# google/supersonic

Hardware: AMD Instinct MI355X
Metric: rows/sec filter->project->aggregate, 100M x 8 INT64/DOUBLE (higher is better)
Workload: dtype int64/f64; 1 GPU; Q-FPA-wide: SUM(a+b),COUNT(*),SUM(c),MIN(d),MAX(d0),SUM(d1),SUM(d2*d3) WHERE a>499 over a device-resident 100000000-row x 8-col block per GPU; rows_per_gpu=100000000, parallelism=single GPU, tile_rows=512, grid=768, lds_bytes=35568, specialized_stages=1

## Files before the change

### supersonic_amd/csrc/launch.h

```cpp
#ifndef SSGPU_LAUNCH_H_
#define SSGPU_LAUNCH_H_

#ifndef __HIPCC_RTC__
#include <hip/hip_runtime_api.h>
#include <stdint.h>
#endif
#include "vm.h"

enum SlotKind {
  SLOT_SUM_INT = 0, SLOT_SUM_DD = 1, SLOT_MIN_U64 = 2, SLOT_MAX_U64 = 3, SLOT_MIN_F64 = 4,
  SLOT_MAX_F64 = 5, SLOT_FIRST = 6, SLOT_LAST = 7, SLOT_COUNT = 8
};
enum EmitKind {
  EMIT_U64 = 0, EMIT_I64KEY = 1, EMIT_U32 = 2, EMIT_I32KEY = 3, EMIT_F64 = 4, EMIT_F32 = 5,
  EMIT_DD_F64 = 6, EMIT_DD_F32 = 7, EMIT_U8 = 8,
  EMIT_DDRES_F64 = 9,
  EMIT_CNT_U64 = 20, EMIT_CNT_U32 = 21,
  EMIT_FKEY_F64 = 100, EMIT_FKEY_F32 = 101
};
#define SSGPU_STATE_ARRAYS 8

struct EmitDesc { void* data; uint8_t* is_null; int slot; int out_kind; };

struct GroupKeyOut { void* data; uint8_t* is_null; uint32_t shift, bits, nullbit, width; };
// ... 129 lines not shown
  const unsigned char* key_nulls[8];
  unsigned int width[8], shift[8], bits[8];
  unsigned int n_keys;
  unsigned int capacity_mask;
  unsigned long long n_rows;
  unsigned long long* keys;
  unsigned int* rows;
  unsigned int* special;
  unsigned int* flags;
  unsigned int* counts;
  unsigned int* slot_of_row;
  unsigned int word[8];
  unsigned long long* keys_hi;
};
hipError_t ssgpu_launch_join_expand(const unsigned int* offsets, const unsigned int* run_start, const unsigned int* rows_sorted,
                                    unsigned long long n_lhs, unsigned long long n_out, unsigned int* lhs_idx, unsigned int* rhs_row, hipStream_t stream);
hipError_t ssgpu_launch_join_build(const JoinBuildParams& P, hipStream_t stream);
hipError_t ssgpu_launch_fill_u32(unsigned int* p, unsigned int v, size_t n, hipStream_t stream);
struct GroupInitParams {
  unsigned long long* keys; unsigned long long n_keys;
  unsigned long long* acc; const unsigned long long* pattern; unsigned int ng; unsigned long long n_acc;
  unsigned int* cnt; unsigned long long n_cnt;
  unsigned int* z[4]; unsigned long long nz[4];
  unsigned int n_rep, pad; unsigned long long rep_stride;
};
hipError_t ssgpu_launch_group_init(const GroupInitParams& P, hipStream_t stream);

hipError_t ssgpu_launch_pipeline(const VmParams& P, int K, int grid, hipStream_t stream);
#ifndef __HIPCC_RTC__
#include <string>
void* ssgpu_rtc_specialize(int device, const VmInstr* prog, int n_instr, int K, bool math, const uint32_t* staged_width, const uint32_t* staged_lds_off,
                           int n_staged, uint32_t static_lds, std::string* why);
hipError_t ssgpu_launch_pipeline_rtc(void* handle, const VmParams& P, int grid, bool static_lds, hipStream_t stream);
void* ssgpu_rtc_specialize_part_agg(int device, const unsigned long long* desc, int n_aggs, unsigned int rec_words, unsigned int n_gaggs, bool any_cnt,
                                    unsigned int lds_bytes, std::string* why, const PlainScatterParams* source = nullptr,
                                    bool dense = false,
                                    bool prefetch = false);
hipError_t ssgpu_launch_group_resident_rtc(void* handle, const PartAggParams& A, const PlainScatterParams& S, int grid, hipStream_t stream);
hipError_t ssgpu_launch_part_agg_rtc(void* handle, const PartAggParams& P, hipStream_t stream);
void* ssgpu_rtc_specialize_pscat(int device, const PlainScatterParams& S, const PscatGeom& g, std::string* why);
hipError_t ssgpu_launch_part_scatter_plain_rtc(void* handle, const PlainScatterParams& P, const PscatGeom& g, int grid, hipStream_t stream);
void* ssgpu_rtc_function(void* handle);
void ssgpu_rtc_release(void* handle);
void ssgpu_rtc_cached_only(bool on);
void ssgpu_rtc_mode(int mode);
int ssgpu_rtc_current_mode();
bool ssgpu_rtc_pending();
void ssgpu_rtc_trim(int keep);
void ssgpu_rtc_stats(long long* modules, long long* code_bytes, long long* compilations, long long* disk_hits);
#endif
hipError_t ssgpu_pipeline_set_max_lds(int bytes);
hipError_t ssgpu_launch_finish_slots(const VmAccRec* partials, int n_slots, int n_parts, const int* slot_kind,
                                     VmAccRec* out, uint64_t* state , hipStream_t stream,
                                     const EmitDesc* descs = nullptr, int n_out = 0 );
hipError_t ssgpu_launch_slots_to_state(const VmAccRec* recs, int n_slots, const int* slot_kind, uint64_t* state,
                                       hipStream_t stream);
hipError_t ssgpu_launch_fold_state(const uint64_t* images, int n_images, uint64_t* state, int n_slots, const int* slot_kind, hipStream_t stream);
hipError_t ssgpu_launch_fold_emit(const uint64_t* images, int n_images, uint64_t* state, int n_slots, const int* slot_kind, VmAccRec* recs,
                                  const EmitDesc* descs, int n_out, hipStream_t stream);
hipError_t ssgpu_launch_state_to_slots(const uint64_t* state, int n_slots, const int* slot_kind, VmAccRec* recs,
                                       hipStream_t stream);
hipError_t ssgpu_launch_emit_scalar(const VmAccRec* recs, const EmitDesc* descs, int n_out, hipStream_t stream);
hipError_t ssgpu_launch_scan_counts(const uint32_t* in, uint32_t* out, int n, uint64_t* total, hipStream_t stream);
hipError_t ssgpu_launch_group_count(const GroupExtractParams& P, uint32_t* tile_counts, hipStream_t stream);
hipError_t ssgpu_launch_group_extract_lb(const GroupExtractParams& P, unsigned long long* status, uint64_t epoch, unsigned int* ctrl, unsigned int* error_flag, hipStream_t stream);
hipError_t ssgpu_launch_group_extract(const GroupExtractParams& P, hipStream_t stream);
hipError_t ssgpu_launch_fill_u64(uint64_t* p, uint64_t v, size_t n, hipStream_t stream);
hipError_t ssgpu_launch_fill_pattern_u64(uint64_t* p, const uint64_t* pattern, uint32_t plen, size_t n,
                                         hipStream_t stream);

hipError_t ssgpu_launch_sort_iota(uint32_t* idx, uint64_t n, hipStream_t s);
hipError_t ssgpu_launch_sort_load_keys(uint64_t* keys, const uint32_t* idx, const void* col, const uint8_t* nulls, uint32_t width,
                                       int kind, int descending, int null_pass, uint64_t n, unsigned long long* bits, hipStream_t s);
uint32_t ssgpu_sort_tiles(uint64_t n);
hipError_t ssgpu_launch_sort_hist(const uint64_t* keys, uint32_t shift, uint64_t n, uint32_t* hist, hipStream_t s);
hipError_t ssgpu_launch_sort_scatter(const uint64_t* keys_in, const uint32_t* idx_in, uint64_t* keys_out, uint32_t* idx_out,
                                     uint32_t shift, uint64_t n, const uint32_t* offsets, hipStream_t s);
hipError_t ssgpu_launch_sort_load_keys_hist(uint64_t* keys, const uint32_t* idx, const void* col, const uint8_t* nulls, uint32_t width, int kind,
                                            int descending, int null_pass, uint64_t n, unsigned long long* bits, uint32_t* hist8, uint32_t* base8, hipStream_t s,
                                            uint64_t* compact_out = nullptr);
hipError_t ssgpu_launch_sort_onesweep(const uint64_t* keys_in, const uint32_t* idx_in, uint64_t* keys_out, uint32_t* idx_out, uint32_t shift, uint64_t n,
                                      const uint32_t* digit_base, unsigned long long* status, uint32_t* ticket, uint64_t epoch, uint32_t* stuck, hipStream_t s);
hipError_t ssgpu_launch_sort_fix_ties(uint64_t* keys, uint32_t* idx, uint64_t n, uint32_t hi_shift, uint32_t* too_long, hipStream_t s);
struct SortRecField { const void* src; void* dst; unsigned int off, width; };
#define SSGPU_SORT_MAX_FIELDS 96
struct SortRecParams { void* recs; unsigned long long n; unsigned int stride, n_fields; SortRecField fields[SSGPU_SORT_MAX_FIELDS]; };
hipError_t ssgpu_launch_sort_pack(const SortRecParams& P, hipStream_t s);
hipError_t ssgpu_launch_sort_gather_rec(const SortRecParams& P, const uint32_t* idx, uint32_t idx_stride, hipStream_t s);
hipError_t ssgpu_launch_sort_fix_ties_compact(uint64_t* kc, const uint64_t* keys, uint64_t n, uint32_t* too_long, hipStream_t s);
hipError_t ssgpu_launch_sort_extract_idx(uint32_t* idx, const uint64_t* kc, uint64_t n, hipStream_t s);
struct UnpackPiece { unsigned long long src_off; void* dst; unsigned long long bytes; };
hipError_t ssgpu_launch_unpack(const char* slab, const UnpackPiece* pieces, unsigned int n_pieces, hipStream_t s);
uint64_t ssgpu_str_scan_partials(uint64_t n);
hipError_t ssgpu_launch_str_scan(uint64_t* data, uint64_t n, uint64_t* partials, hipStream_t s);
hipError_t ssgpu_launch_str_hash(const uint8_t* bytes, const uint64_t* offs, const uint8_t* nulls, uint64_t n, uint64_t* hashes, hipStream_t s);
hipError_t ssgpu_launch_str_insert(const uint8_t* bytes, const uint64_t* offs, const uint8_t* nulls, const uint64_t* hashes, uint64_t n,
                                   uint64_t* table, uint64_t cap, uint32_t* row_slot, uint32_t* error, hipStream_t s);
hipError_t ssgpu_launch_str_compact(const uint64_t* table, uint64_t cap, const uint8_t* bytes, const uint64_t* offs, uint32_t* count,
                                    uint32_t* d_slot, uint64_t* d_off, uint64_t* d_len, uint64_t* d_key, uint32_t* d_idx, hipStream_t s);
hipError_t ssgpu_launch_str_sort(uint64_t* d_key, uint32_t* d_idx, uint64_t d, uint64_t p, const uint8_t* bytes, const uint64_t* d_off,
                                 const uint64_t* d_len, hipStream_t s);
hipError_t ssgpu_launch_str_rank(const uint32_t* d_idx, const uint32_t* d_slot, const uint64_t* d_len, uint64_t d, int32_t* slot_rank,
                                 uint64_t* out_len, hipStream_t s);
hipError_t ssgpu_launch_str_codes(const uint32_t* row_slot, const uint8_t* nulls, const int32_t* slot_rank, uint64_t n, int32_t* codes, hipStream_t s);
hipError_t ssgpu_launch_str_gather(const uint8_t* bytes, const uint64_t* d_off, const uint32_t* d_idx, const uint64_t* out_off, uint64_t d,
                                   uint8_t* out, hipStream_t s);
hipError_t ssgpu_launch_str_recode(const int32_t* src, const uint8_t* nulls, const int32_t* remap, int32_t n_remap, uint64_t n, int32_t* dst,
// ... 47 lines not shown
```

### supersonic_amd/csrc/pipeline_kernels.hip

```cpp
#ifndef __HIPCC_RTC__
#include <hip/hip_runtime.h>
#include <stdint.h>
#endif
#include "vm.h"
#include "launch.h"
#ifdef SSGPU_RTC_NINSTR
#include "rtc_prog.h"
#endif

typedef unsigned long long u64;
typedef long long i64;
typedef unsigned int u32;
typedef int i32;
typedef unsigned char u8;

#ifdef SSGPU_PC_PROFILE
#define PC_PROF(...) __VA_ARGS__
#else
#define PC_PROF(...)
#endif
struct LdsBase {
  __device__ __forceinline__ char* operator+(u32 off) const {
    return (char*)(__attribute__((address_space(3))) char*)off;
  }
// ... 679 lines not shown
        case SLOT_COUNT: v0 = cnt; break;
        case SLOT_SUM_INT: v0 = wave_reduce_u64(F0[s], [](u64 x, u64 y) { return x + y; }); break;
        case SLOT_MIN_U64: v0 = wave_reduce_u64(F0[s], [](u64 x, u64 y) { return x < y ? x : y; }); break;
        case SLOT_MAX_U64: v0 = wave_reduce_u64(F0[s], [](u64 x, u64 y) { return x > y ? x : y; }); break;
        case SLOT_MIN_F64: v0 = wave_reduce_u64(F0[s], [](u64 x, u64 y) { return u2d(y) < u2d(x) ? y : x; }); break;
        case SLOT_MAX_F64: v0 = wave_reduce_u64(F0[s], [](u64 x, u64 y) { return u2d(x) < u2d(y) ? y : x; }); break;
        case SLOT_SUM_DD: {
          DD d; d.hi = u2d(F0[s]); d.lo = u2d(F1[s]);
          d = wave_reduce_dd(d); v0 = d2u(d.hi); v1 = d2u(d.lo);
        } break;
        case SLOT_FIRST: case SLOT_LAST: {
          const bool first = kind == SLOT_FIRST;
          const u64 trow = first ? wave_reduce_u64(F1[s], [](u64 x, u64 y) { return x < y ? x : y; })
                                 : wave_reduce_u64(FC[s] ? F1[s] : 0ull, [](u64 x, u64 y) { return x > y ? x : y; });
          const u64 owner = __ballot(FC[s] != 0 && F1[s] == trow);
          const int src = owner ? __ffsll((long long)owner) - 1 : 0;
          v0 = readlane64(F0[s], src); v1 = trow;
        } break;
        default: break;
      }
      if (lane == 0) { VmAccRec* A = acc_rec(P, (u32)s, wave); A->v0 = v0; A->v1 = v1; A->cnt = cnt; A->pad = 0; }
    }
  }

  __syncthreads();
  for (int s = t; s < P.n_slots; s += VM_COMPUTE_THREADS)
    for (int w = 0; w < VM_WAVES; ++w)
      P.wg_partials[((size_t)blockIdx.x * P.n_slots + s) * VM_WAVES + w] = *acc_rec(P, (u32)s, w);
}
#endif

#ifndef __HIPCC_RTC__

__device__ __forceinline__ void combine_rec(int kind, VmAccRec& acc, const VmAccRec& r) {
  if (r.cnt == 0) return;
  switch (kind) {
    case SLOT_COUNT:
    case SLOT_SUM_INT: acc.v0 += r.v0; break;
    case SLOT_SUM_DD: {
      DD a; a.hi = u2d(acc.v0); a.lo = u2d(acc.v1);
      DD b; b.hi = u2d(r.v0); b.lo = u2d(r.v1);
      a = dd_add(a, b); acc.v0 = d2u(a.hi); acc.v1 = d2u(a.lo);
    } break;
    case SLOT_MIN_U64: acc.v0 = acc.cnt ? (r.v0 < acc.v0 ? r.v0 : acc.v0) : r.v0; break;
    case SLOT_MAX_U64: acc.v0 = acc.cnt ? (r.v0 > acc.v0 ? r.v0 : acc.v0) : r.v0; break;
    case SLOT_MIN_F64: acc.v0 = acc.cnt ? (u2d(r.v0) < u2d(acc.v0) ? r.v0 : acc.v0) : r.v0; break;
    case SLOT_MAX_F64: acc.v0 = acc.cnt ? (u2d(acc.v0) < u2d(r.v0) ? r.v0 : acc.v0) : r.v0; break;
    case SLOT_FIRST: if (!acc.cnt || r.v1 < acc.v1) { acc.v0 = r.v0; acc.v1 = r.v1; } break;
    case SLOT_LAST: if (!acc.cnt || r.v1 >= acc.v1) { acc.v0 = r.v0; acc.v1 = r.v1; } break;
  }
  acc.cnt += r.cnt;
}

__device__ __forceinline__ void slot_to_state(const VmAccRec r, int kind, int s, int n_slots, u64* __restrict__ state) {
  u64* sum_i = state; u64* cnt = state + n_slots; u64* hi = state + 2 * n_slots; u64* lo = state + 3 * n_slots;
  u64* mn = state + 4 * n_slots; u64* mx = state + 5 * n_slots;
  u64* mnf = state + 6 * n_slots; u64* mxf = state + 7 * n_slots;
  const bool fl = kind == SLOT_FIRST || kind == SLOT_LAST;
  sum_i[s] = (kind == SLOT_SUM_INT || kind == SLOT_COUNT || fl) ? r.v0 : 0;
  cnt[s] = r.cnt;
  hi[s] = kind == SLOT_SUM_DD ? r.v0 : d2u(0.0);
  lo[s] = kind == SLOT_SUM_DD ? r.v1 : d2u(0.0);
  mn[s] = (kind == SLOT_MIN_U64 && r.cnt) ? (r.v0 ^ 0x8000000000000000ull) : (kind == SLOT_FIRST && r.cnt) ? (r.v1 ^ 0x8000000000000000ull) : 0x7FFFFFFFFFFFFFFFull;
  mx[s] = (kind == SLOT_MAX_U64 && r.cnt) ? (r.v0 ^ 0x8000000000000000ull) : (kind == SLOT_LAST && r.cnt) ? (r.v1 ^ 0x8000000000000000ull) : 0x8000000000000000ull;
  mnf[s] = (kind == SLOT_MIN_F64 && r.cnt) ? r.v0 : d2u(__builtin_inf());
  mxf[s] = (kind == SLOT_MAX_F64 && r.cnt) ? r.v0 : d2u(-__builtin_inf());
}
__device__ __forceinline__ VmAccRec state_to_slot(const u64* __restrict__ state, int kind, int s, int n_slots) {
  VmAccRec r; r.v0 = 0; r.v1 = 0; r.pad = 0;
  r.cnt = state[n_slots + s];
  switch (kind) {
    case SLOT_COUNT: case SLOT_SUM_INT: r.v0 = state[s]; break;
    case SLOT_SUM_DD: {
      DD a; a.hi = u2d(state[2 * n_slots + s]); a.lo = 0.0;
      a = dd_add_d(a, u2d(state[3 * n_slots + s]));
      r.v0 = d2u(a.hi); r.v1 = d2u(a.lo);
    } break;
    case SLOT_MIN_U64: r.v0 = state[4 * n_slots + s] ^ 0x8000000000000000ull; break;
    case SLOT_MAX_U64: r.v0 = state[5 * n_slots + s] ^ 0x8000000000000000ull; break;
    case SLOT_MIN_F64: r.v0 = state[6 * n_slots + s]; break;
    case SLOT_MAX_F64: r.v0 = state[7 * n_slots + s]; break;
    case SLOT_FIRST: r.v0 = state[s]; r.v1 = state[4 * n_slots + s] ^ 0x8000000000000000ull; break;
    case SLOT_LAST: r.v0 = state[s]; r.v1 = state[5 * n_slots + s] ^ 0x8000000000000000ull; break;
    default: break;
  }
  return r;
}

__device__ __forceinline__ void emit_scalar_one(const EmitDesc d, const VmAccRec r);
__global__ __launch_bounds__(256) void ssgpu_finish_slots_kernel(const VmAccRec* __restrict__ partials, int n_slots,
                                                                 int n_parts, const int* __restrict__ slot_kind,
                                                                 VmAccRec* __restrict__ out, u64* __restrict__ state,
                                                                 const EmitDesc* __restrict__ descs, int n_out) {
  __shared__ VmAccRec tree[256];
  const int s = blockIdx.x, t = threadIdx.x;
  const int kind = slot_kind[s];
  VmAccRec acc; acc.v0 = 0; acc.v1 = 0; acc.cnt = 0; acc.pad = 0;
  if (kind == SLOT_SUM_DD) { acc.v0 = d2u(-0.0); acc.v1 = d2u(0.0); }
  for (int i = t; i < n_parts; i += 256) {
    const VmAccRec r = partials[((size_t)(i / VM_WAVES) * n_slots + s) * VM_WAVES + (i % VM_WAVES)];
    combine_rec(kind, acc, r);
  }
  tree[t] = acc;
  __syncthreads();
  for (int stride = 128; stride > 0; stride >>= 1) {
    if (t < stride) { VmAccRec a = tree[t]; combine_rec(kind, a, tree[t + stride]); tree[t] = a; }
    __syncthreads();
  }
  if (t == 0) { out[s] = tree[0]; if (state) slot_to_state(tree[0], kind, s, n_slots, state); }
  if (descs)
    for (int i = t; i < n_out; i += 256) { const EmitDesc d = descs[i]; if (d.slot == s) emit_scalar_one(d, tree[0]); }
}

__global__ void ssgpu_slots_to_state_kernel(const VmAccRec* __restrict__ recs, int n_slots,
                                            const int* __restrict__ slot_kind, u64* __restrict__ state) {
  int s = blockIdx.x * blockDim.x + threadIdx.x;
  if (s >= n_slots) return;
  slot_to_state(recs[s], slot_kind[s], s, n_slots, state);
}
__global__ void ssgpu_state_to_slots_kernel(const u64* __restrict__ state, int n_slots,
                                            const int* __restrict__ slot_kind, VmAccRec* __restrict__ recs) {
  int s = blockIdx.x * blockDim.x + threadIdx.x;
  if (s >= n_slots) return;
  recs[s] = state_to_slot(state, slot_kind[s], s, n_slots);
}


__device__ __forceinline__ void emit_value(void* dst, size_t idx, int out_kind, u64 v0, u64 v1) {
  switch (out_kind) {
    case EMIT_U64: reinterpret_cast<u64*>(dst)[idx] = v0; break;
    case EMIT_I64KEY: reinterpret_cast<i64*>(dst)[idx] = unkey_i64(v0); break;
    case EMIT_U32: reinterpret_cast<u32*>(dst)[idx] = (u32)v0; break;
    case EMIT_I32KEY: reinterpret_cast<i32*>(dst)[idx] = (i32)unkey_i64(v0); break;
    case EMIT_F64: reinterpret_cast<double*>(dst)[idx] = u2d(v0); break;
    case EMIT_F32: reinterpret_cast<float*>(dst)[idx] = (float)u2d(v0); break;
    case EMIT_DD_F64: { double hi = u2d(v0), lo = u2d(v1);
      reinterpret_cast<double*>(dst)[idx] = (lo == 0.0) ? hi : hi + lo; } break;
    case EMIT_DDRES_F64: { const double hi = u2d(v0), lo = u2d(v1), sm = hi + lo, bp = sm - hi;
      reinterpret_cast<double*>(dst)[idx] = (lo == 0.0) ? 0.0 : (hi - (sm - bp)) + (lo - bp); } break;
    case EMIT_DD_F32: { double hi = u2d(v0), lo = u2d(v1);
      reinterpret_cast<float*>(dst)[idx] = (float)((lo == 0.0) ? hi : hi + lo); } break;
    case EMIT_U8: reinterpret_cast<u8*>(dst)[idx] = (u8)(v0 != 0); break;
    default: break;
  }
}


__device__ __forceinline__ void emit_scalar_one(const EmitDesc d, const VmAccRec r) {
  if (d.out_kind == EMIT_CNT_U64 || d.out_kind == EMIT_CNT_U32)
    emit_value(d.data, 0, d.out_kind == EMIT_CNT_U64 ? EMIT_U64 : EMIT_U32, r.cnt, 0);
  else
    emit_value(d.data, 0, d.out_kind, r.v0, r.v1);
  if (d.is_null) d.is_null[0] = r.cnt == 0;
}
__global__ void ssgpu_emit_scalar_kernel(const VmAccRec* __restrict__ recs, const EmitDesc* __restrict__ descs,
                                         int n_out) {
  int i = blockIdx.x * blockDim.x + threadIdx.x;
  if (i >= n_out) return;
  const EmitDesc d = descs[i];
  emit_scalar_one(d, recs[d.slot]);
}

__global__ __launch_bounds__(1024) void ssgpu_scan_counts_kernel(const u32* __restrict__ in, u32* __restrict__ out,
                                                                  int n, u64* __restrict__ total) {
// ... 878 lines not shown
  }
  u64 bits;
  if (fam == 2) {
    const double tr = trunc(vf);
    bits = (tr >= -9223372036854775808.0 && tr < 9223372036854775808.0) ? (u64)(i64)tr : 0x8000000000000000ull;
  } else bits = fam == 1 ? vu : (u64)vi;
  if (dst_kind == 2 || dst_kind == 3) reinterpret_cast<u64*>(dst)[i] = bits;
  else if (dst_kind == 0 || dst_kind == 1) reinterpret_cast<u32*>(dst)[i] = (u32)bits;
  else reinterpret_cast<u8*>(dst)[i] = (u8)bits;
}
hipError_t ssgpu_launch_gather_rowid(void* dst, const uint8_t* dst_null, const void* src, uint32_t width, int src_kind, int dst_kind, const uint64_t* rowids, uint64_t rowid_mask,
                                     int64_t row_id_base, const uint64_t* n_rows_dev, uint64_t n_rows_max, hipStream_t stream) {
  if (n_rows_max) hipLaunchKernelGGL(ssgpu_gather_rowid_kernel, dim3((unsigned)((n_rows_max + 255) / 256)), dim3(256), 0, stream,
                                     dst, dst_null, src, width, src_kind, dst_kind, (const u64*)rowids, (u64)rowid_mask, (i64)row_id_base, (const u64*)n_rows_dev, (u64)n_rows_max);
  return hipGetLastError();
}
hipError_t ssgpu_launch_fill_u32(unsigned int* p, unsigned int v, size_t n, hipStream_t stream) {
  if (n) hipLaunchKernelGGL(ssgpu_fill_u32_kernel, dim3((unsigned)std::min<size_t>((n + 255) / 256, 4096)), dim3(256), 0, stream, p, v, n);
  return hipGetLastError();
}
hipError_t ssgpu_launch_part_agg(const PartAggParams& P, unsigned int lds_bytes, hipStream_t stream) {
  if (P.rec_words <= 8) hipLaunchKernelGGL(ssgpu_part_agg_kernel<8>, dim3(P.n_parts), dim3(SSGPU_PART_THREADS), lds_bytes, stream, P);
  else if (P.rec_words <= 16) hipLaunchKernelGGL(ssgpu_part_agg_kernel<16>, dim3(P.n_parts), dim3(SSGPU_PART_THREADS), lds_bytes, stream, P);
  else if (P.rec_words <= SSGPU_PART_MAX_WORDS) hipLaunchKernelGGL(ssgpu_part_agg_kernel<SSGPU_PART_MAX_WORDS>, dim3(P.n_parts), dim3(SSGPU_PART_THREADS), lds_bytes, stream, P);
  else return hipErrorInvalidValue;
  return hipGetLastError();
}
hipError_t ssgpu_launch_group_resident(const PartAggParams& P, const PlainScatterParams& S, unsigned int lds_bytes, int grid, hipStream_t stream) {
  if (P.rec_words <= 8) hipLaunchKernelGGL(ssgpu_group_resident_kernel<8>, dim3(grid), dim3(SSGPU_PART_THREADS), lds_bytes, stream, P, S);
  else hipLaunchKernelGGL(ssgpu_group_resident_kernel<16>, dim3(grid), dim3(SSGPU_PART_THREADS), lds_bytes, stream, P, S);
  return hipGetLastError();
}
hipError_t ssgpu_part_agg_set_max_lds(int bytes) {
  hipError_t e = hipFuncSetAttribute(reinterpret_cast<const void*>(ssgpu_part_agg_kernel<8>), hipFuncAttributeMaxDynamicSharedMemorySize, bytes);
  if (e != hipSuccess) return e;
  e = hipFuncSetAttribute(reinterpret_cast<const void*>(ssgpu_group_resident_kernel<8>), hipFuncAttributeMaxDynamicSharedMemorySize, bytes);
  if (e != hipSuccess) return e;
  e = hipFuncSetAttribute(reinterpret_cast<const void*>(ssgpu_group_resident_kernel<16>), hipFuncAttributeMaxDynamicSharedMemorySize, bytes);
  if (e != hipSuccess) return e;
  e = hipFuncSetAttribute(reinterpret_cast<const void*>(ssgpu_part_agg_kernel<SSGPU_PART_MAX_WORDS>), hipFuncAttributeMaxDynamicSharedMemorySize, bytes);
  if (e != hipSuccess) return e;
  return hipFuncSetAttribute(reinterpret_cast<const void*>(ssgpu_part_agg_kernel<16>), hipFuncAttributeMaxDynamicSharedMemorySize, bytes);
}
hipError_t ssgpu_pipeline_set_max_lds(int bytes) {
  hipError_t e;
  e = hipFuncSetAttribute(reinterpret_cast<const void*>(ssgpu_pipeline_kernel<1, false>), hipFuncAttributeMaxDynamicSharedMemorySize, bytes); if (e != hipSuccess) return e;
  e = hipFuncSetAttribute(reinterpret_cast<const void*>(ssgpu_pipeline_kernel<2, false>), hipFuncAttributeMaxDynamicSharedMemorySize, bytes); if (e != hipSuccess) return e;
  e = hipFuncSetAttribute(reinterpret_cast<const void*>(ssgpu_pipeline_kernel<4, false>), hipFuncAttributeMaxDynamicSharedMemorySize, bytes); if (e != hipSuccess) return e;
  e = hipFuncSetAttribute(reinterpret_cast<const void*>(ssgpu_pipeline_kernel<1, true>), hipFuncAttributeMaxDynamicSharedMemorySize, bytes); if (e != hipSuccess) return e;
  e = hipFuncSetAttribute(reinterpret_cast<const void*>(ssgpu_pipeline_kernel<2, true>), hipFuncAttributeMaxDynamicSharedMemorySize, bytes); if (e != hipSuccess) return e;
  e = hipFuncSetAttribute(reinterpret_cast<const void*>(ssgpu_pipeline_kernel<4, true>), hipFuncAttributeMaxDynamicSharedMemorySize, bytes);
  return e;
}
hipError_t ssgpu_launch_finish_slots(const VmAccRec* partials, int n_slots, int n_parts, const int* slot_kind,
                                     VmAccRec* out, uint64_t* state, hipStream_t stream, const EmitDesc* descs, int n_out) {
  hipLaunchKernelGGL(ssgpu_finish_slots_kernel, dim3(n_slots), dim3(256), 0, stream, partials, n_slots, n_parts, slot_kind, out, (u64*)state, descs, n_out);
  return hipGetLastError();
}
hipError_t ssgpu_launch_slots_to_state(const VmAccRec* recs, int n_slots, const int* slot_kind, uint64_t* state, hipStream_t stream) {
  int blocks = (n_slots + 63) / 64;
  hipLaunchKernelGGL(ssgpu_slots_to_state_kernel, dim3(blocks), dim3(64), 0, stream, recs, n_slots, slot_kind, (u64*)state);
  return hipGetLastError();
}
__device__ __forceinline__ void fold_state_slot(const u64* __restrict__ images, int n_images, u64* __restrict__ state, int n_slots, int kind, int s);
__global__ __launch_bounds__(64) void ssgpu_fold_state_kernel(const u64* __restrict__ images, int n_images, u64* __restrict__ state,
                                                              int n_slots, const int* __restrict__ slot_kind) {
  const int s = blockIdx.x * 64 + threadIdx.x;
  if (s >= n_slots) return;
  fold_state_slot(images, n_images, state, n_slots, slot_kind[s], s);
}
__device__ __forceinline__ void fold_state_slot(const u64* __restrict__ images, int n_images, u64* __restrict__ state, int n_slots, int kind, int s) {
  const size_t total = (size_t)SSGPU_STATE_ARRAYS * n_slots;
  u64 a[SSGPU_STATE_ARRAYS];
  for (int k = 0; k < SSGPU_STATE_ARRAYS; ++k) a[k] = images[(size_t)k * n_slots + s];
  for (int r = 1; r < n_images; ++r) {
    u64 v[SSGPU_STATE_ARRAYS];
    for (int k = 0; k < SSGPU_STATE_ARRAYS; ++k) v[k] = images[(size_t)r * total + (size_t)k * n_slots + s];
    if (kind == SLOT_FIRST) { if ((i64)v[4] < (i64)a[4]) a[0] = v[0]; }
    else if (kind == SLOT_LAST) { if ((i64)v[5] > (i64)a[5]) a[0] = v[0]; }
    else a[0] += v[0];
    a[1] += v[1];
    a[2] = d2u(u2d(a[2]) + u2d(v[2]));
    a[3] = d2u(u2d(a[3]) + u2d(v[3]));
    a[4] = (i64)v[4] < (i64)a[4] ? v[4] : a[4];
    a[5] = (i64)v[5] > (i64)a[5] ? v[5] : a[5];
    a[6] = u2d(v[6]) < u2d(a[6]) ? v[6] : a[6];
    a[7] = u2d(v[7]) > u2d(a[7]) ? v[7] : a[7];
  }
  for (int k = 0; k < SSGPU_STATE_ARRAYS; ++k) state[(size_t)k * n_slots + s] = a[k];
}
__global__ __launch_bounds__(256) void ssgpu_fold_emit_kernel(const u64* __restrict__ images, int n_images, u64* __restrict__ state, int n_slots,
                                                              const int* __restrict__ slot_kind, VmAccRec* __restrict__ recs,
                                                              const EmitDesc* __restrict__ descs, int n_out) {
  for (int s = threadIdx.x; s < n_slots; s += 256) {
    fold_state_slot(images, n_images, state, n_slots, slot_kind[s], s);
    recs[s] = state_to_slot(state, slot_kind[s], s, n_slots);
  }
  __threadfence_block();
  __syncthreads();
  for (int i = threadIdx.x; i < n_out; i += 256) { const EmitDesc d = descs[i]; emit_scalar_one(d, recs[d.slot]); }
}
hipError_t ssgpu_launch_fold_emit(const uint64_t* images, int n_images, uint64_t* state, int n_slots, const int* slot_kind, VmAccRec* recs,
                                  const EmitDesc* descs, int n_out, hipStream_t stream) {
  hipLaunchKernelGGL(ssgpu_fold_emit_kernel, dim3(1), dim3(256), 0, stream, (const u64*)images, n_images, (u64*)state, n_slots, slot_kind, recs, descs, n_out);
  return hipGetLastError();
}
hipError_t ssgpu_launch_fold_state(const uint64_t* images, int n_images, uint64_t* state, int n_slots, const int* slot_kind, hipStream_t stream) {
  if (n_slots > 0) hipLaunchKernelGGL(ssgpu_fold_state_kernel, dim3((n_slots + 63) / 64), dim3(64), 0, stream, (const u64*)images, n_images, (u64*)state, n_slots, slot_kind);
  return hipGetLastError();
// ... 94 lines not shown
```

### supersonic_amd/csrc/runtime.cpp

```cpp
#include <hip/hip_runtime_api.h>

#include <atomic>
#include <map>
#include <mutex>
#include <stdio.h>
#include <string.h>
#include <algorithm>
#include <cmath>
#include <string>
#include <unistd.h>
#include <thread>
#include <unordered_set>
#include <vector>
#include <deque>
#include <functional>

#include "engine.h"

using namespace ssgpu;

#define HIP_TRY(ctx, expr)                                                          \
  do {                                                                               \
    hipError_t _e = (expr);                                                          \
    if (_e != hipSuccess) {                                                          \
// ... 177 lines not shown
  std::vector<VmInstr> host_prog_main;
  std::string rtc_why;
  ProgramLayout lay{};
  ProgramLayout lay_count{};
  int n_instr_main = 0, n_instr_count = 0;
  int grid = 0;
  DevBuf wg_partials, slot_recs, slot_kind, emit_descs, state;
  DevBuf tile_counts, tile_offsets, total;
  DevBuf xstatus; uint64_t x_epoch = 0;
  DevBuf gkeys, gacc, gcnt, goverflow, gpattern, gmergeop;
  int group_wgs = 3;
  bool group_local = true;
  int group_sub = 1;
  bool group_partitioned = false;
  uint32_t part_n = 256;
  bool part_n_chosen = false;
  bool part_slab_failed = false;
  bool scouted = false;
  int64_t scout_full_rows = 0;
  bool part_slab = false;
  double part_groups_est = 0;
  uint32_t part_seg_growth = 1;
  bool part_failed = false;
  DevBuf prog_pscatter, part_hist, part_recs;
  ProgramLayout lay_pscatter{};
  int n_instr_pscatter = 0;
  RtcSlot rtc_pscatter; std::vector<VmInstr> host_prog_pscatter;
  RtcSlot rtc_plain;
  RtcSlot rtc_part;
  RtcSlot rtc_resident;
  RtcSlot rtc_hot;
  uint32_t hot_n = 0; uint64_t hot_keys[SSGPU_HOT_MAX] = {0};
  int64_t hot_sampled_run = -1;
  DevBuf hot_out;
  struct DenseState {
    bool on = false, failed = false, checked = false, fixed = false, resident = false;
    uint32_t n_keys = 0, n_chunks = 1;
    uint64_t lo[8] = {0}, hi[8] = {0};
    uint32_t span[8] = {0}, stride[8] = {0};
    uint64_t slots = 0;
    uint32_t np = 0, cap = 0;
    uint64_t chunk_bytes = 0;
    int64_t widened = 0;
  } dense;
  DevBuf dense_dom, dense_flags;
  void* dense_table = nullptr;
  std::vector<DevBuf> rowid_tmp;
  std::vector<DevBuf> jkeys, jkeys_hi, jrows, jmisc;
  std::vector<DevBuf> jcounts, jstarts, jslot_of_row, jrows_sorted;
  DevBuf jx_offsets, jx_lhs_idx, jx_rhs_row;
  std::vector<VmJoin> vm_joins;
  uint32_t capacity = 0;
  DevBuf error_flag;
  DevBuf debug, debug_pc, total2;
  DevBuf skeys_a, skeys_b, skeys_c, sidx_a, sidx_b, shist, soffs, seg_id, sstatus, sticket, srecs, dflag;
  DevBuf rank_first, rank_of_seg, rank_row, rank_own;
  DevBuf seg_counts, seg_offsets, seg_total;
  DevBuf route_scratch;
  uint64_t sort_epoch = 0;
  bool emit_ready = false;
  bool emitted_with_finish = false;
  bool pattern_ready = false;
  DevBuf out_arena;
  std::vector<OutCol> out;
  int64_t out_rows = -1;
  const void* out_rows_dev = nullptr;
  int64_t out_capacity = 0;
  int last_group_shape = 0;
  int last_reruns = 0;
  int last_sort_passes = 0, last_sort_mode = 0;
  bool last_plain_scatter = false;
  PinnedBuf fb_host;
  int fb_pending = 0;
  hipEvent_t fb_event = nullptr;
  int steady = 0;
  uint32_t steady_bypass = 0;
};

struct ssgpu_result {
  ssgpu_plan* plan = nullptr;
  std::vector<PinnedBuf> host_data, host_nulls;
  std::vector<bool> fetched;
  std::vector<ssgpu_dict*> concat_dicts;
  ~ssgpu_result() { for (ssgpu_dict* d : concat_dicts) if (d) ssgpu_dict_destroy(d); }
};

struct ssgpu_plan {
  ssgpu_ctx* ctx = nullptr;
  MemQuota quota;
  int64_t expr_row_capacity = INT64_MAX;
  PlanDesc desc;
  std::vector<Stage> stages;
  std::vector<StageExec> exec;
  Schema result_schema;
  std::vector<std::string> attr_names;
  std::vector<ssgpu_column> aux_cols;
  int64_t aux_rows = -1;
  std::string describe, describe_full;
  std::atomic<int> interrupted{0};
  int64_t n_runs = 0;
  bool specialize = false;
  bool cached_only = false;
  bool best_effort = false; int64_t be_cut = -1, be_capacity = 0, be_window = 0, be_base = 0, be_window_fail = 0;
  uint32_t group_capacity_hint = 0;
  bool lazy_feedback = false;
  bool background = false;
// ... 940 lines not shown
    switch (kind) {
      case SLOT_SUM_DD: memcpy(&i0, &nzero, 8); break;
      case SLOT_MIN_U64: i0 = ~0ull; break;
      case SLOT_MIN_F64: memcpy(&i0, &pinf, 8); break;
      case SLOT_MAX_F64: memcpy(&i0, &ninf, 8); break;
      case SLOT_FIRST: i1 = ~0ull; break;
      default: break;
    }
    P->slot_init0[i] = i0; P->slot_init1[i] = i1; P->slot_kind[i] = kind;
  }
}

int distinct_flags(ssgpu_ctx* c, const Stage& st, StageExec& ex, const InCols& in, ssgpu_column* out) {
  const uint32_t nk = (uint32_t)st.distinct_cols.size();
  if (nk > 16) { c->err = "DISTINCT aggregate under more than 15 group keys"; return SSGPU_ERROR_NOT_IMPLEMENTED; }
  const void* kdata[16] = {nullptr}; const uint8_t* knulls[16] = {nullptr}; uint32_t kwidth[16] = {0};
  for (uint32_t k = 0; k < nk; ++k) {
    const int col = st.distinct_cols[k];
    kdata[k] = in.cols[col].data; knulls[k] = in.cols[col].is_null; kwidth[k] = (uint32_t)dtype_width(st.in_schema[col].dtype);
  }
  HIP_TRY(c, ex.dflag.ensure((size_t)std::max<int64_t>(in.rows, 1)));
  HIP_TRY(c, ssgpu_launch_cluster_flags(kdata, knulls, kwidth, nk, (uint64_t)in.rows, ex.dflag.as<uint8_t>(), c->stream));
  out->data = ex.dflag.p; out->is_null = nullptr;
  return SSGPU_OK;
}

int prepare_scalar_emit(ssgpu_plan* p, size_t si, int* n_out);
int run_scalar_agg(ssgpu_plan* p, size_t si, const InCols& in0, int64_t row_id_base, bool stop_at_partial) {
  ssgpu_ctx* c = p->ctx; Stage& st = p->stages[si]; StageExec& ex = p->exec[si];
  InCols in = in0;
  if (!st.distinct_cols.empty()) {
    ssgpu_column f; const int rc = distinct_flags(c, st, ex, in0, &f); if (rc != SSGPU_OK) return rc;
    in.cols.push_back(f);
  }
  VmParams P;
  fill_params(&P, st.main, ex.lay, ex.prog_main, ex.n_instr_main, in, row_id_base);
  apply_joins(p, ex, st.main, &P);
  if (c->tile_map >= 2) P.flags |= VM_FLAG_XCD_CHUNKS;
  fill_fast_slots(&P, st);
  const int grid = grid_for(c, ex.lay, P.n_tiles);
  ex.grid = grid;
  const int ns = st.main.n_slots;
  HIP_TRY(c, ex.wg_partials.ensure((size_t)grid * ns * VM_WAVES * sizeof(VmAccRec)));
  HIP_TRY(c, ex.slot_recs.ensure((size_t)ns * sizeof(VmAccRec)));
  HIP_TRY(c, ex.state.ensure((size_t)ns * SSGPU_STATE_ARRAYS * sizeof(uint64_t)));
  if (!ex.slot_kind.p) {
    std::vector<int> kinds((size_t)ns, SLOT_COUNT);
    for (size_t i = 0; i < st.aggs.size(); ++i)
      if (st.aggs[i].slot == (int)i) kinds[i] = st.aggs[i].slot_kind;
    HIP_TRY(c, ex.slot_kind.ensure(kinds.size() * sizeof(int)));
    HIP_TRY(c, hipMemcpy(ex.slot_kind.p, kinds.data(), kinds.size() * sizeof(int), hipMemcpyHostToDevice));
  }
  P.wg_partials = ex.wg_partials.as<VmAccRec>();
  P.error_flag = ex.error_flag.as<unsigned int>();
  if (c->debug_timing) {
    HIP_TRY(c, ex.debug.ensure((size_t)grid * 4 * 8));
    P.debug = ex.debug.as<unsigned long long>();
  }
  { int rc = attach_pc_profile(c, ex, &P); if (rc != SSGPU_OK) return rc; }
  if (c->profile) HIP_TRY(c, hipEventRecord(p->ev_dom0, c->stream));
  HIP_TRY(c, launch_main(p, st, ex, P, ex.lay.K, grid));
  if (c->profile) HIP_TRY(c, hipEventRecord(p->ev_dom1, c->stream));
  { int rc = print_pc_profile(c, ex, st.main, P.n_instr); if (rc != SSGPU_OK) return rc; }
  int n_emit = 0;
  ex.emitted_with_finish = false;
  if (!stop_at_partial && c->fuse_emit) { const int rc = prepare_scalar_emit(p, si, &n_emit); if (rc != SSGPU_OK) return rc; ex.emitted_with_finish = true; }
  HIP_TRY(c, ssgpu_launch_finish_slots(ex.wg_partials.as<VmAccRec>(), ns, grid * VM_WAVES, ex.slot_kind.as<int>(),
                                       ex.slot_recs.as<VmAccRec>(), stop_at_partial ? ex.state.as<uint64_t>() : nullptr, c->stream,
                                       ex.emitted_with_finish ? ex.emit_descs.as<EmitDesc>() : nullptr, n_emit));
  p->counters.n_launches += 2;
  p->counters.tile_rows = P.tile_rows; p->counters.grid = grid; p->counters.lds_bytes = (int32_t)ex.lay.lds_bytes;
  if (c->debug_timing) {
    std::vector<unsigned long long> dbg((size_t)grid * 4);
    HIP_TRY(c, hipMemcpy(dbg.data(), ex.debug.p, dbg.size() * 8, hipMemcpyDeviceToHost));
    double tot = 0, wait = 0, tiles = 0;
    for (int g = 0; g < grid; ++g) { tot += (double)dbg[g * 4]; wait += (double)dbg[g * 4 + 1]; tiles += (double)dbg[g * 4 + 2]; }
    fprintf(stderr, "[ssgpu debug] grid=%d tiles/wg=%.1f cycles/wg=%.0f wait=%.1f%% cycles/tile=%.0f (wait %.0f)\n", grid, tiles / grid,
            tot / grid, 100.0 * wait / tot, tot / tiles, wait / tiles);
  }
  return SSGPU_OK;
}

static const int64_t kSeqSumPiece = 1 << 21;
static int run_seq_sums(ssgpu_plan* p, Stage& st, StageExec& ex, const InCols& in, const uint32_t* seg_id) {
  ssgpu_ctx* c = p->ctx;
  auto kind_of = [](int dtype) {
    switch (dtype) {
      case SSGPU_INT32: return 0; case SSGPU_UINT32: return 1; case SSGPU_INT64: return 2; case SSGPU_UINT64: return 3;
      case SSGPU_FLOAT: return 4; default: return 5;
    }
  };
  for (auto& q : st.seq_sums) {
    const void* src = in.cols[q.in_col].data;
    const uint8_t* src_nulls = st.in_schema[q.in_col].nullable ? in.cols[q.in_col].is_null : nullptr;
    uint8_t* dst_nulls = ex.out[q.out_col].nullable ? ex.out[q.out_col].nulls.as<uint8_t>() : nullptr;
    const int sk = kind_of(st.in_schema[q.in_col].dtype), dk = kind_of(st.out_schema[q.out_col].dtype);
    if (seg_id || in.rows <= kSeqSumPiece) {
      HIP_TRY(c, ssgpu_launch_seq_sum(src, src_nulls, sk, seg_id, (uint64_t)in.rows, ex.out[q.out_col].data.p, dst_nulls, dk, c->stream));
      p->counters.n_launches += 1;
      continue;
    }
    HIP_TRY(c, ex.total2.ensure(16));
    for (int64_t first = 0; first < in.rows; first += kSeqSumPiece) {
      const int64_t end = std::min<int64_t>(in.rows, first + kSeqSumPiece);
      HIP_TRY(c, ssgpu_launch_seq_sum(src, src_nulls, sk, nullptr, (uint64_t)end, ex.out[q.out_col].data.p, dst_nulls, dk, c->stream,
                                      (uint64_t)first, ex.total2.as<uint64_t>(), first > 0 ? 1 : 0));
      p->counters.n_launches += 1;
      if (end < in.rows) {
        HIP_TRY(c, hipStreamSynchronize(c->stream));
        if (p->interrupted.exchange(0)) { c->err = "interrupted"; return SSGPU_INTERRUPTED; }
      }
    }
  }
  return SSGPU_OK;
}

int prepare_scalar_emit(ssgpu_plan* p, size_t si, int* n_out) {
  ssgpu_ctx* c = p->ctx; Stage& st = p->stages[si]; StageExec& ex = p->exec[si];
  int rc = ensure_out_cols(c, st, ex, 1);
  if (rc != SSGPU_OK) return rc;
  *n_out = (int)st.aggs.size();
  if (!ex.emit_ready) {
// ... 1354 lines not shown
  int rc = run_plan(p, cols.data(), (int32_t)cols.size(), p->last_rows, p->last_base, false);
  if (rc != SSGPU_OK) return rc;
  rc = settle_plan(p);
  if (rc != SSGPU_OK) return rc;
  rc = check_error_flags(p);
  p->nan_seen = false;
  return rc;
}

int run_plan(ssgpu_plan* p, const ssgpu_column* cols, int32_t n_cols, int64_t rows, int64_t row_id_base, bool partial) {
  ssgpu_ctx* c = p->ctx;
  if (!c || c->device < 0) { if (c) c->err = "no gfx950 device bound to this context (bind-only context)"; return SSGPU_ERROR_NO_DEVICE; }
  ssgpu_rtc_mode(!p->cached_only ? 0 : p->background && rows >= p->background_min_rows ? 2 : 1);
  p->run_row_end = row_id_base + rows;
  p->nan_seen = false;
  if (p->deferred) {
    p->deferred = false;
    for (auto& ex : p->exec) {
      if (!ex.fb_pending) continue;
      if (ex.fb_event) HIP_TRY(c, hipEventSynchronize(ex.fb_event)); else HIP_TRY(c, hipStreamSynchronize(c->stream));
      const uint32_t* fb = static_cast<const uint32_t*>(ex.fb_host.p);
      const int kind = ex.fb_pending; ex.fb_pending = 0;
      if (fb[0] || (kind == 2 && (fb[1] || fb[3]))) ex.steady = 0;
      else if (kind == 1 && (uint64_t)fb[1] > 2ull * ex.steady_bypass + (uint64_t)(p->last_rows >> 6)) ex.steady = 0;
    }
  }
  if (n_cols != (int)p->desc.input_schema.size()) { c->err = "column count does not match the plan's input schema"; return SSGPU_ERROR_ATTRIBUTE_COUNT_MISMATCH; }
  if (rows < 0) { c->err = "negative row count"; return SSGPU_ERROR_INVALID_ARGUMENT_VALUE; }
  if (p->interrupted.exchange(0)) { c->err = "interrupted"; return SSGPU_INTERRUPTED; }
  QuotaScope quota_scope(&p->quota);
  HIP_TRY(c, hipSetDevice(c->device));
  { const int orc = order_after_uploads(c); if (orc != SSGPU_OK) return orc; }
  memset(&p->counters, 0, sizeof(p->counters));
  p->counters.rows_in = rows;
  p->result.fetched.assign(p->result.fetched.size(), false);
  for (ssgpu_dict*& cd : p->result.concat_dicts) { if (cd) ssgpu_dict_destroy(cd); cd = nullptr; }
  InCols in; in.cols.assign(cols, cols + n_cols); in.rows = rows;
  if (partial && !(p->stages.size() == 1 && p->stages[0].kind == STAGE_SCALAR_AGG)) {
    c->err = "partial runs need a plan whose only stage is a ScalarAggregate"; return SSGPU_ERROR_NOT_IMPLEMENTED;
  }
  for (size_t si = 0; si < p->stages.size(); ++si) {
    if (si == 0) ++p->n_runs;
    int rc = prepare_stage(p, si);
    if (rc != SSGPU_OK) return rc;
  }
  if (c->profile) {
    const int slot = (int)(p->profiled_runs % ssgpu_plan::kEventRing);
    if (!p->ring0[slot]) { HIP_TRY(c, hipEventCreate(&p->ring0[slot])); HIP_TRY(c, hipEventCreate(&p->ring1[slot])); g_events.fetch_add(2); }
    p->ev_dom0 = p->ring0[slot]; p->ev_dom1 = p->ring1[slot];
    ++p->profiled_runs;
    p->events_valid = false;
    if (c->profile_total) HIP_TRY(c, hipEventRecord(p->ev_begin, c->stream));
  }
  for (size_t si = 0; si < p->exec.size(); ++si)
    if (p->exec[si].error_flag.p && !p->keep_error_flags && !(si == 0 && p->stages[si].kind == STAGE_GROUP_AGG)) HIP_TRY(c, hipMemsetAsync(p->exec[si].error_flag.p, 0, sizeof(uint32_t), c->stream));
  int64_t alg_bytes = 0;
  for (size_t si = 0; si < p->stages.size(); ++si) {
    if (p->interrupted.exchange(0)) { c->err = "interrupted"; return SSGPU_INTERRUPTED; }
    Stage& st = p->stages[si];
    int rc = SSGPU_OK;
    alg_bytes += st.algorithmic_bytes_per_row * in.rows;
    rc = build_joins(p, st, p->exec[si]);
    if (rc != SSGPU_OK) return rc;
    switch (st.kind) {
      case STAGE_SCALAR_AGG:
        rc = run_scalar_agg(p, si, in, row_id_base, partial);
        if (rc == SSGPU_OK && !partial) rc = emit_scalar_agg(p, si);
        if (rc == SSGPU_OK && !partial && !st.seq_sums.empty()) rc = run_seq_sums(p, st, p->exec[si], in, nullptr);
        break;
      case STAGE_MATERIALIZE: rc = run_materialize(p, si, in, row_id_base); break;
      case STAGE_GROUP_AGG: rc = run_group_agg(p, si, in, row_id_base); break;
      case STAGE_SORT: rc = run_sort(p, si, in); break;
      case STAGE_CLUSTERS: rc = run_clusters(p, si, in, row_id_base); break;
      case STAGE_JOIN_EXPAND: rc = run_join_expand(p, si, in); break;
      case STAGE_FOLD_TAIL: rc = run_fold_tail(p, si, in); break;
      default: c->err = "stage kind not executable yet"; rc = SSGPU_ERROR_NOT_IMPLEMENTED; break;
    }
    if (rc != SSGPU_OK) return rc;
    if (si + 1 < p->stages.size()) {
      StageExec& ex = p->exec[si];
      const Stage& nx = p->stages[si + 1];
      const bool device_rows = c->async_handoff != 0 && !c->debug_timing && ex.out_rows < 0 && ex.out_capacity > 0 && nx.kind == STAGE_MATERIALIZE &&
                               !nx.has_filter && nx.distinct_cols.empty() && !nx.has_segment && !nx.has_rank && nx.joins.empty();
      int64_t r = 0;
      in.rows_dev = nullptr;
      if (device_rows) {
        r = ex.out_capacity;
        in.rows_dev = static_cast<const unsigned long long*>(rows_word(ex));
      } else {
        rc = stage_rows(p, si, &r);
        if (rc != SSGPU_OK) return rc;
        rc = check_error_flags(p);
        if (rc != SSGPU_OK) return rc;
      }
      in.cols.clear();
      for (auto& oc : ex.out) { ssgpu_column col; col.data = oc.data.p; col.is_null = oc.nullable ? oc.nulls.as<uint8_t>() : nullptr; in.cols.push_back(col); }
      in.rows = r;
      row_id_base = 0;
    }
  }
  if (c->profile && c->profile_total) { HIP_TRY(c, hipEventRecord(p->ev_end, c->stream)); p->events_valid = true; }
  p->counters.algorithmic_bytes = alg_bytes;
  p->last_rows = rows;
  p->last_cols.assign(cols, cols + n_cols); p->last_base = row_id_base; p->last_partial = partial;
  p->partial_pending = partial;
  return SSGPU_OK;
}

// ... 1364 lines not shown
```

Baseline: 99.89 billion rows/s.

## Fold error-flag reset into finish kernel and batch partial loads in slot reduction

The scalar-aggregate path now has the main kernel write errors into a separate work word. The finish kernel atomically swaps that word to zero and publishes it to the user-visible error flag. This removes the per-run hipMemsetAsync of the error flag, which was a separate stream operation before the aggregate launch. The finish kernel also replaces its strided per-thread loop with an 8-wide batched load-then-combine chain to expose more memory-level parallelism. The cost is an extra atomic exchange, added state-handoff complexity between runs, and a changed launcher signature.

```diff
diff --git a/supersonic_amd/csrc/launch.h b/supersonic_amd/csrc/launch.h
--- a/supersonic_amd/csrc/launch.h
+++ b/supersonic_amd/csrc/launch.h
@@ -205,7 +205,8 @@
 hipError_t ssgpu_pipeline_set_max_lds(int bytes);
 hipError_t ssgpu_launch_finish_slots(const VmAccRec* partials, int n_slots, int n_parts, const int* slot_kind,
                                      VmAccRec* out, uint64_t* state , hipStream_t stream,
-                                     const EmitDesc* descs = nullptr, int n_out = 0 );
+                                     const EmitDesc* descs, int n_out ,
+                                     unsigned int* err_work, unsigned int* err_pub, unsigned int keep_errors );
 hipError_t ssgpu_launch_slots_to_state(const VmAccRec* recs, int n_slots, const int* slot_kind, uint64_t* state,
                                        hipStream_t stream);
 hipError_t ssgpu_launch_fold_state(const uint64_t* images, int n_images, uint64_t* state, int n_slots, const int* slot_kind, hipStream_t stream);
diff --git a/supersonic_amd/csrc/pipeline_kernels.hip b/supersonic_amd/csrc/pipeline_kernels.hip
--- a/supersonic_amd/csrc/pipeline_kernels.hip
+++ b/supersonic_amd/csrc/pipeline_kernels.hip
@@ -755,6 +755,24 @@
   acc.cnt += r.cnt;
 }
 
+__device__ __forceinline__ VmAccRec fold_chain(int kind, const VmAccRec* first, size_t stride, int n) {
+  VmAccRec acc; acc.v0 = 0; acc.v1 = 0; acc.cnt = 0; acc.pad = 0;
+  if (kind == SLOT_SUM_DD) { acc.v0 = d2u(-0.0); acc.v1 = d2u(0.0); }
+  for (int j0 = 0; j0 < n; j0 += 8) {
+    VmAccRec r[8];
+#pragma unroll
+    for (int q = 0; q < 8; ++q) r[q] = first[(size_t)(j0 + q < n ? j0 + q : n - 1) * stride];
+#pragma unroll
+    for (int q = 0; q < 8; ++q)
+      if (j0 + q < n) combine_rec(kind, acc, r[q]);
+  }
+  return acc;
+}
+__device__ __forceinline__ void publish_error_word(unsigned int* work, unsigned int* pub, u32 keep) {
+  const u32 e = atomicExch(work, 0u);
+  if (keep) { if (e) atomicOr(pub, e); }
+  else __hip_atomic_store(pub, e, __ATOMIC_RELAXED, __HIP_MEMORY_SCOPE_AGENT);
+}
 __device__ __forceinline__ void slot_to_state(const VmAccRec r, int kind, int s, int n_slots, u64* __restrict__ state) {
   u64* sum_i = state; u64* cnt = state + n_slots; u64* hi = state + 2 * n_slots; u64* lo = state + 3 * n_slots;
   u64* mn = state + 4 * n_slots; u64* mx = state + 5 * n_slots;
@@ -794,17 +812,13 @@
 __global__ __launch_bounds__(256) void ssgpu_finish_slots_kernel(const VmAccRec* __restrict__ partials, int n_slots,
                                                                  int n_parts, const int* __restrict__ slot_kind,
                                                                  VmAccRec* __restrict__ out, u64* __restrict__ state,
-                                                                 const EmitDesc* __restrict__ descs, int n_out) {
+                                                                 const EmitDesc* __restrict__ descs, int n_out,
+                                                                 unsigned int* err_work, unsigned int* err_pub, u32 keep_errors) {
   __shared__ VmAccRec tree[256];
   const int s = blockIdx.x, t = threadIdx.x;
   const int kind = slot_kind[s];
-  VmAccRec acc; acc.v0 = 0; acc.v1 = 0; acc.cnt = 0; acc.pad = 0;
-  if (kind == SLOT_SUM_DD) { acc.v0 = d2u(-0.0); acc.v1 = d2u(0.0); }
-  for (int i = t; i < n_parts; i += 256) {
-    const VmAccRec r = partials[((size_t)(i / VM_WAVES) * n_slots + s) * VM_WAVES + (i % VM_WAVES)];
-    combine_rec(kind, acc, r);
-  }
-  tree[t] = acc;
+  tree[t] = fold_chain(kind, &partials[((size_t)(t / VM_WAVES) * n_slots + s) * VM_WAVES + (t % VM_WAVES)],
+                       (size_t)(256 / VM_WAVES) * n_slots * VM_WAVES, t < n_parts ? (n_parts - t + 255) / 256 : 0);
   __syncthreads();
   for (int stride = 128; stride > 0; stride >>= 1) {
     if (t < stride) { VmAccRec a = tree[t]; combine_rec(kind, a, tree[t + stride]); tree[t] = a; }
@@ -813,6 +827,7 @@
   if (t == 0) { out[s] = tree[0]; if (state) slot_to_state(tree[0], kind, s, n_slots, state); }
   if (descs)
     for (int i = t; i < n_out; i += 256) { const EmitDesc d = descs[i]; if (d.slot == s) emit_scalar_one(d, tree[0]); }
+  if (s == 0 && t == 0 && err_pub) publish_error_word(err_work, err_pub, keep_errors);
 }
 
 __global__ void ssgpu_slots_to_state_kernel(const VmAccRec* __restrict__ recs, int n_slots,
@@ -1797,9 +1812,9 @@
   e = hipFuncSetAttribute(reinterpret_cast<const void*>(ssgpu_pipeline_kernel<4, true>), hipFuncAttributeMaxDynamicSharedMemorySize, bytes);
   return e;
 }
-hipError_t ssgpu_launch_finish_slots(const VmAccRec* partials, int n_slots, int n_parts, const int* slot_kind,
-                                     VmAccRec* out, uint64_t* state, hipStream_t stream, const EmitDesc* descs, int n_out) {
-  hipLaunchKernelGGL(ssgpu_finish_slots_kernel, dim3(n_slots), dim3(256), 0, stream, partials, n_slots, n_parts, slot_kind, out, (u64*)state, descs, n_out);
+hipError_t ssgpu_launch_finish_slots(const VmAccRec* partials, int n_slots, int n_parts, const int* slot_kind, VmAccRec* out, uint64_t* state,
+                                     hipStream_t stream, const EmitDesc* descs, int n_out, unsigned int* err_work, unsigned int* err_pub, unsigned int keep_errors) {
+  hipLaunchKernelGGL(ssgpu_finish_slots_kernel, dim3(n_slots), dim3(256), 0, stream, partials, n_slots, n_parts, slot_kind, out, (u64*)state, descs, n_out, err_work, err_pub, keep_errors);
   return hipGetLastError();
 }
 hipError_t ssgpu_launch_slots_to_state(const VmAccRec* recs, int n_slots, const int* slot_kind, uint64_t* state, hipStream_t stream) {
diff --git a/supersonic_amd/csrc/runtime.cpp b/supersonic_amd/csrc/runtime.cpp
--- a/supersonic_amd/csrc/runtime.cpp
+++ b/supersonic_amd/csrc/runtime.cpp
@@ -253,6 +253,7 @@
   std::vector<VmJoin> vm_joins;
   uint32_t capacity = 0;
   DevBuf error_flag;
+  DevBuf error_work;
   DevBuf debug, debug_pc, total2;
   DevBuf skeys_a, skeys_b, skeys_c, sidx_a, sidx_b, shist, soffs, seg_id, sstatus, sticket, srecs, dflag;
   DevBuf rank_first, rank_of_seg, rank_row, rank_own;
@@ -1299,7 +1300,12 @@
     HIP_TRY(c, hipMemcpy(ex.slot_kind.p, kinds.data(), kinds.size() * sizeof(int), hipMemcpyHostToDevice));
   }
   P.wg_partials = ex.wg_partials.as<VmAccRec>();
-  P.error_flag = ex.error_flag.as<unsigned int>();
+  if (!ex.error_work.p) {
+    HIP_TRY(c, ex.error_work.ensure(sizeof(uint32_t)));
+    HIP_TRY(c, hipMemsetAsync(ex.error_work.p, 0, sizeof(uint32_t), c->stream));
+    HIP_TRY(c, hipMemsetAsync(ex.error_flag.p, 0, sizeof(uint32_t), c->stream));
+  }
+  P.error_flag = ex.error_work.as<unsigned int>();
   if (c->debug_timing) {
     HIP_TRY(c, ex.debug.ensure((size_t)grid * 4 * 8));
     P.debug = ex.debug.as<unsigned long long>();
@@ -1314,7 +1320,8 @@
   if (!stop_at_partial && c->fuse_emit) { const int rc = prepare_scalar_emit(p, si, &n_emit); if (rc != SSGPU_OK) return rc; ex.emitted_with_finish = true; }
   HIP_TRY(c, ssgpu_launch_finish_slots(ex.wg_partials.as<VmAccRec>(), ns, grid * VM_WAVES, ex.slot_kind.as<int>(),
                                        ex.slot_recs.as<VmAccRec>(), stop_at_partial ? ex.state.as<uint64_t>() : nullptr, c->stream,
-                                       ex.emitted_with_finish ? ex.emit_descs.as<EmitDesc>() : nullptr, n_emit));
+                                       ex.emitted_with_finish ? ex.emit_descs.as<EmitDesc>() : nullptr, n_emit,
+                                       ex.error_work.as<unsigned int>(), ex.error_flag.as<unsigned int>(), p->keep_error_flags ? 1u : 0u));
   p->counters.n_launches += 2;
   p->counters.tile_rows = P.tile_rows; p->counters.grid = grid; p->counters.lds_bytes = (int32_t)ex.lay.lds_bytes;
   if (c->debug_timing) {
@@ -2775,8 +2782,10 @@
     p->events_valid = false;
     if (c->profile_total) HIP_TRY(c, hipEventRecord(p->ev_begin, c->stream));
   }
-  for (size_t si = 0; si < p->exec.size(); ++si)
-    if (p->exec[si].error_flag.p && !p->keep_error_flags && !(si == 0 && p->stages[si].kind == STAGE_GROUP_AGG)) HIP_TRY(c, hipMemsetAsync(p->exec[si].error_flag.p, 0, sizeof(uint32_t), c->stream));
+  for (size_t si = 0; si < p->exec.size(); ++si) {
+    const int kind = p->stages[si].kind;
+    if (p->exec[si].error_flag.p && !p->keep_error_flags && !(si == 0 && (kind == STAGE_GROUP_AGG || kind == STAGE_SCALAR_AGG))) HIP_TRY(c, hipMemsetAsync(p->exec[si].error_flag.p, 0, sizeof(uint32_t), c->stream));
+  }
   int64_t alg_bytes = 0;
   for (size_t si = 0; si < p->stages.size(); ++si) {
     if (p->interrupted.exchange(0)) { c->err = "interrupted"; return SSGPU_INTERRUPTED; }
```

New measurement: 100.0 billion rows/s (median of 6 runs). About the same (+0.1%).
